# rvp-group/srrg2_slam_interfaces

Measured on AMD Instinct MI355X. Metric: icp_iterations_per_sec, higher is better.
Workload: dtype f32; 1 GPU; C2: SE(3) point-to-plane AlignerSlice, 100000-pt synthetic cloud pair per GPU, 10 ICP iterations per compute(), gated NN 0.25 m + normal gate, Cauchy 0.05; points=100000, alignments_total=1, all_success=True, last_status=0, last_num_inliers=99432, parallelism=single GPU

## Files before the change

srrg2_slam_interfaces_amd/csrc/aligner_host.hip:

```cpp
#include <algorithm>
#include <cmath>
#include <cstdio>
#include <cstdlib>
#include <chrono>
#include <cstring>
#include <string>
#include <vector>

#include "det_math.h"
#include "kernels.h"

#include "host_util.h"

namespace srrg2amd {
thread_local std::string g_err;
int fail(int code, const std::string& msg) {
  g_err = msg;
  return code;
}
}

namespace {

using srrg2amd::DevBuf;
// ... 802 lines not shown
      const Slice* sfc = a->slices[fc];
      const int sl     = tn.search_lists;
      const bool lists = sl >= 2 || (sl == 1 && K > 4) || (sl < 0 && (K > 4 || sfc->grid_computes >= 1 || sfc->lists_tried));
      small            = !lists && max_nm <= 384;
    }
  }
  const int fast_from = tn.fast_from_iteration;
  bool fuse = false;
  auto fast_ppt_of = [&](int k_launch) {
    return tn.fast_points_per_thread > 0 ? tn.fast_points_per_thread : (k_launch >= (fuse ? 16 : 64) ? 2 : 1);
  };
  const int fast_min = tn.fast_min_points;
  const bool fast_gather = tn.fast_gather >= 0 ? tn.fast_gather != 0 : K > 4;
  const bool fast_batch_queue = tn.fast_batch_queue != 0;
  const int lds_tile = pairs ? 0 : (tn.lds_tile >= 0 ? tn.lds_tile : (K > 4 ? 1 : 0));
  const int search_lists = tn.search_lists;
  const int search_team_knob = tn.search_team;
  std::vector<char> cnl((size_t) std::max(nslices, 1), 0);
  std::vector<SliceDev> sdev((size_t) nslices);
  int first_cue = -1;
  for (int si = 0; si < nslices; ++si) {
    Slice* s     = a->slices[si];
    SliceCtl& sc = C.slices[si];
    sc.kind                     = s->cfg.kind;
    sc.min_num_correspondences  = s->cfg.min_num_correspondences;
    sc.robust_kind              = s->cfg.robustifier;
    sc.robust_thr               = s->cfg.robustifier_chi_threshold;
    sc.gate                     = s->cfg.finder_max_distance;
    sc.has_prior                = s->has_prior ? 1 : 0;
    sc.prior_sets_initial_guess = s->cfg.prior_sets_initial_guess;
    std::memcpy(sc.prior_Z, s->prior_Z, sizeof(sc.prior_Z));
    std::memcpy(sc.prior_info, s->cfg.prior_information_diag, sizeof(sc.prior_info));
    sc.partials  = nullptr;
    sc.finder    = s->cfg.finder;
    sc.K0        = s->cfg.camera_matrix[0];
    sc.K4        = s->cfg.camera_matrix[4];
    sc.umax      = proj_extent(s->cfg.image_cols, s->cfg.camera_matrix[2]);
    sc.vmax      = proj_extent(s->cfg.image_rows, s->cfg.camera_matrix[5]);
    sc.depth_min = s->cfg.depth_min;
    sc.pinf_bits = nullptr;
    sc.ninf_bits = nullptr;
    if (s->cfg.kind == SRRG2_SLICE_PRIOR) continue;
    if (first_cue < 0) first_cue = si;
    int nm_max_s = 0;
    for (int k = 0; k < K; ++k) nm_max_s = std::max(nm_max_s, all[(size_t) si * K + k].nm);
    const int queue_min = tn.queue_min_points;
    const bool want_lists = search_lists >= 2 || (search_lists == 1 && K > 4) ||
                            (search_lists < 0 && (K > 4 || s->grid_computes >= 1 || s->lists_tried));
    if (!pairs) s->grid_computes++;
    if (s->cfg.finder == SRRG2_FINDER_NN_GATED && !small && want_lists && !pairs) {
      if ((rc = ensure_lists(a, s, 96LL << 20))) return rc;
      cnl[(size_t) si] = s->grid.list_R > 0 ? 1 : 0;
    }
    const bool use_queue = s->cfg.finder == SRRG2_FINDER_NN_GATED && nm_max_s >= queue_min && K <= 4 && !small && !cnl[(size_t) si] && !pairs;
    const bool fast_queue = s->cfg.finder == SRRG2_FINDER_NN_GATED && K > 4 && !small && fast_batch_queue && !pairs;
    s->fast_queue_only = fast_queue && !use_queue;
    const int nblocks    = PARTIAL_SLOTS;
    {
      const size_t cap_before = s->partials.cap;
      if ((rc = s->partials.reserve((size_t) 3 * K * nblocks * ACC_N))) return rc;
      if (s->partials.cap != cap_before) s->slots_zeroed = 0;
    }
    if (use_queue || fast_queue) {
      if ((rc = s->queue.reserve((size_t) std::max(s->nm_total, 1) * 10))) return rc;
      if ((rc = s->qcount.reserve((size_t) 2 * K))) return rc;
    }
    sc.qcount = (use_queue || fast_queue) ? s->qcount.p : nullptr;
    sc.qprobe_host = nullptr;
    sc.probs       = nullptr;
    if (use_queue) {
      if ((rc = ensure_pinned(s->qprobe_host, s->qprobe_cap, (size_t) 2 * K))) return rc;
      std::memset(s->qprobe_host, 0x7f, sizeof(int) * (size_t) 2 * K);
      sc.qprobe_host = s->qprobe_host;
      sc.probs       = a->probs.p + (size_t) si * K;
    }
    sc.partials  = s->partials.p;
    sc.pinf_bits = s->pinf.p;
    sc.ninf_bits = pairs ? a->pair_rows.p + PAIR_ROW_NINF : s->scalars.p + 7;
    sc.finf_bits = s->scalars.p + 10;
    sc.gcorr_off = nullptr;
    sc.nm_global = (a->reduce_fn && s->cfg.kind != SRRG2_SLICE_PRIOR) ? (int) a->shard_total : 0;
    SliceDev& d       = sdev[si];
    d.grid            = pairs ? GridDev{} : s->grid;
    d.mpts            = s->moving.p;
    d.mnrm            = s->moving_has_normals ? s->moving_nrm.p : nullptr;
    d.corr_fixed      = s->corr_fixed.p;
    d.corr_resp       = s->corr_resp.p;
    d.corr_stat       = s->corr_stat.p;
    d.prev_n          = s->prev_n.p;
    d.prev_pos        = s->prev_pos.p;
    d.prev_f          = s->prev_f.p;
    d.prev_m          = s->prev_m.p;
    d.dbg             = nullptr;
    if (!a->timeline_path.empty()) {
      const size_t nw = (size_t) K * ((nm_max_s + 255) / 256) * 4;
      if ((rc = s->dbg.reserve(32 * nw * 16))) return rc;
      HIP_TRY(hipMemsetAsync(s->dbg.p, 0, 32 * nw * 16 * sizeof(unsigned long long), a->stream));
      d.dbg = s->dbg.p;
    }
    d.partials        = s->partials.p;
    d.queue           = (use_queue || fast_queue) ? (void*) s->queue.p : nullptr;
    d.qcount          = (use_queue || fast_queue) ? s->qcount.p : nullptr;
    d.slice_idx       = si;
    d.robust_kind     = s->cfg.robustifier;
    d.robust_thr      = s->cfg.robustifier_chi_threshold;
    d.normal_cos      = s->cfg.finder_normal_cos;
    d.use_normal_gate = (s->cfg.finder_normal_cos > -1.f && (pairs ? a->pair_normals : s->fixed_has_normals) && s->moving_has_normals) ? 1 : 0;
    d.gather_prev     = (s->cfg.finder == SRRG2_FINDER_NN_GATED && fast_gather) ? 1 : 0;
    d.variable_kind   = a->kind;
    d.finder          = s->cfg.finder;
    d.factor          = s->cfg.kind;
    std::memcpy(d.K, s->cfg.camera_matrix, sizeof(d.K));
    d.rows            = s->cfg.image_rows;
    d.cols            = s->cfg.image_cols;
    d.depth_min       = s->cfg.depth_min;
    d.depth_max       = s->cfg.depth_max;
    d.gate            = s->cfg.finder_max_distance;
    d.fixed_org       = s->fixed_raw.p;
    d.fixed_org_nrm   = s->fixed_has_normals ? s->fixed_nrm_raw.p : nullptr;
    d.zbuf            = nullptr;
    d.zbuf_parity     = 0;
    d.gcorr = nullptr; d.gcorr_off = nullptr; d.gcorr_stat = nullptr;
    d.moving_raw      = s->moving_raw.p;
    if (s->cfg.finder == SRRG2_FINDER_CORRESPONDENCES) {
      if ((int) s->h_gcorr_off.size() != K + 1)
        return fail(SRRG2_E_STATE, "compute: given-correspondences slice without correspondences for every alignment");
      if (s->cfg.kind == SRRG2_SLICE_P2PLANE && !s->fixed_has_normals)
        return fail(SRRG2_E_STATE, "compute: point-to-plane slice without fixed normals");
      const int total = s->h_gcorr_off[(size_t) K];
      for (int k = 0; k < K; ++k) {
        const int nmk = all[(size_t) si * K + k].nm;
        for (int c = s->h_gcorr_off[(size_t) k]; c < s->h_gcorr_off[(size_t) k + 1]; ++c)
          if (s->h_gcorr[(size_t) c].fixed_idx < 0 || s->h_gcorr[(size_t) c].fixed_idx >= s->nf ||
              s->h_gcorr[(size_t) c].moving_idx < 0 || s->h_gcorr[(size_t) c].moving_idx >= nmk)
            return fail(SRRG2_E_INVALID, "compute: correspondence index out of range");
      }
      if ((rc = s->gcorr.reserve((size_t) std::max(total, 1)))) return rc;
      if ((rc = s->gcorr_off.reserve((size_t) K + 1))) return rc;
      if ((rc = s->gcorr_stat.reserve((size_t) std::max(total, 1)))) return rc;
      if (total > 0)
        HIP_TRY(hipMemcpyAsync(s->gcorr.p, s->h_gcorr.data(), sizeof(srrg2_correspondence) * (size_t) total,
                               hipMemcpyHostToDevice, a->stream));
      HIP_TRY(hipMemcpyAsync(s->gcorr_off.p, s->h_gcorr_off.data(), sizeof(int) * ((size_t) K + 1), hipMemcpyHostToDevice,
                             a->stream));
      HIP_TRY(hipStreamSynchronize(a->stream));
      d.gcorr      = s->gcorr.p;
      d.gcorr_off  = s->gcorr_off.p;
      d.gcorr_stat = s->gcorr_stat.p;
      sc.gcorr_off = s->gcorr_off.p;
    }
    if (s->cfg.finder == SRRG2_FINDER_PROJECTIVE) {
      if ((rc = s->zbuf.reserve((size_t) 2 * K * d.rows * d.cols))) return rc;
      d.zbuf = s->zbuf.p;
      HIP_TRY(hipMemsetAsync(s->zbuf.p, 0xff, (size_t) 2 * K * d.rows * d.cols * sizeof(unsigned long long), a->stream));
    }
    if (a->dim == 3)
      dm::se3_inverse(s->cfg.sensor_in_robot, d.Sinv);
    else
      dm::se2_inverse(s->cfg.sensor_in_robot, d.Sinv);
    std::memcpy(sc.Sinv, d.Sinv, sizeof(sc.Sinv));
  }
  if (K > 1 && first_cue >= 0 && !slice_offsets) {
    for (int si = 0; si < nslices; ++si)
      if (a->slices[si]->cfg.kind != SRRG2_SLICE_PRIOR && si != first_cue)
        return fail(SRRG2_E_UNSUPPORTED, "compute_batch supports one cue slice (plus prior slices)");
  }
// ... 1544 lines not shown
```

srrg2_slam_interfaces_amd/csrc/device_types.h:

```cpp
#pragma once
#include <hip/hip_runtime.h>
#include <stdint.h>

#include "../../include/srrg2_slam_amd.h"

#define ACC_N 32
#define PARTIAL_SLOTS 32
#define ACC_B 21
#define ACC_CHI_IN 27
#define ACC_CHI_OUT 28
#define ACC_N_IN 29
#define ACC_N_OUT 30
#define ACC_N_CORR 31
#define TERM_WINDOW_MAX 64
#define NO_MATCH 0x7fffffff

__host__ __device__ __forceinline__ constexpr int hidx(int a, int b) {
  return a * 6 - (a * (a - 1)) / 2 + (b - a);
}

struct GridDev {
  float ox, oy, oz;
  float h, inv_h;
  int nx, ny, nz;
  int rmax;
  int rfar_gate;
  float gate2;
  float gate2_ext;
  int n;
  const int* cell_start;
  const float4* pts;
  const float4* nrm;
  const int* pos_of;
  int list_R;
  const struct GridLists* lists;
};
struct GridLists {
  int R;
  int lnx, lny, lnz;
  const int* start;
  const uint4* ent;
  float cls_b2[14];
};
#define CNL_MAX_R 3
#ifndef CNL_ENTRY_MAX
#define CNL_ENTRY_MAX 16
#endif
#define CNL_MAX_CLASS 12

#define PUB_SLICE_GRANULES 64
#define PUB_G_KEXP 24
#define PUB_G_FLAGS 25
#define PUB_G_NSTATS 26
#define PUB_G_WCOUNT 27
#define PUB_G_NPASSES 28
#define PUB_G_X 32
#define PUB_FLAG_STOP 1u
#define PUB_FLAG_PHASE1 2u
#define PUB_FLAG_PRIOR 4u
#define PUB_EPOCH_REPLICAS 8
#define PUB_EPOCH_STRIDE 32
struct CtlParams;
struct FusedCtl {
  unsigned long long* pub;
  unsigned* pub_epoch;
  const CtlParams* ctl;
  srrg2_iteration_stats* stats;
  long long* prev_partials;
  long long* zero_partials;
  int epoch;
  int min_num_correspondences;
  int max_stats;
  int has_term;
  int first_round;
  int prior;
  int prior_mask;
  int nslices;
};

struct SliceDev {
  GridDev grid;
  const float4* mpts;
  const float4* mnrm;
  int* corr_fixed;
  float* corr_resp;
  uint8_t* corr_stat;
  float4* prev_f;
  float4* prev_n;
  int* prev_pos;
  float* prev_m;
  long long* partials;
  void* queue;
  int* qcount;
  int slice_idx;
  int robust_kind;
  float robust_thr;
  float normal_cos;
  int use_normal_gate;
  int gather_prev;
  int variable_kind;
  int finder;
  int factor;
  float K[9];
  int rows, cols;
  float depth_min, depth_max;
  float gate;
  const float4* fixed_org;
  const float4* fixed_org_nrm;
  unsigned long long* zbuf;
  int zbuf_parity;
  const srrg2_correspondence* gcorr;
  const int* gcorr_off;
  uint8_t* gcorr_stat;
  const float4* moving_raw;
  unsigned long long* dbg;
  int prob0;
  float Sinv[12];
// ... 99 lines not shown
```

srrg2_slam_interfaces_amd/csrc/kernels.hip:

```cpp
#include <cstdlib>
#include <algorithm>

#include "kernels.h"

#include <type_traits>

#include "det_math.h"

#include "device_util.h"

namespace {

#define FX_MAGIC 6755399441055744.0
#define FX_MAGIC_BITS 0x4338000000000000ll
__device__ __forceinline__ long long fx_bits(double biased) { return __double_as_longlong(biased) - FX_MAGIC_BITS; }

__device__ __forceinline__ unsigned long long key_min(unsigned long long a, unsigned long long b) {
  double r;
  asm("v_min_f64 %0, %1, %2" : "=v"(r) : "v"(__longlong_as_double((long long) a)), "v"(__longlong_as_double((long long) b)));
  return (unsigned long long) __double_as_longlong(r);
}

template <int DIM>
__device__ __forceinline__ float cand_d2(const float4 f, float qx, float qy, float qz) {
// ... 471 lines not shown

namespace {

#ifndef SRRG2_CNL_REDEAL
#define SRRG2_CNL_REDEAL 0
#endif
#ifdef SRRG2_CNL_STATS
__device__ unsigned long long g_cnl_stats[4 * 16];
#define CNL_STAT(k, v)                                                                                   \
  do {                                                                                                   \
    const unsigned long long v_ = (unsigned long long) (v);    \
    if ((threadIdx.x & 63) == 0) atomicAdd(&g_cnl_stats[(stat_it < 3 ? stat_it : 3) * 16 + (k)], v_);    \
  } while (0)
#else
#define CNL_STAT(k, v) do { } while (0)
#endif
constexpr int CNL_POOL = 512;

struct CnlWave {
  uint2 pool[CNL_POOL];
  unsigned long long key[64];
  unsigned b2[64];
  float q[3][64];
};

template <int DIM>
__device__ __forceinline__ void test_group_glb(const float4* __restrict__ pts, int j, int cnt, float qx, float qy, float qz,
                                               unsigned long long& bkey, float& b2) {
  if (cnt > 0) {
    const float4 a0 = pts[j], a1 = pts[j + 1], a2 = pts[j + 2], a3 = pts[j + 3];
    const float d0 = cand_d2<DIM>(a0, qx, qy, qz);
    float d1 = cand_d2<DIM>(a1, qx, qy, qz), d2 = cand_d2<DIM>(a2, qx, qy, qz), d3 = cand_d2<DIM>(a3, qx, qy, qz);
    unsigned i1 = (unsigned) __float_as_int(a1.w), i2 = (unsigned) __float_as_int(a2.w), i3 = (unsigned) __float_as_int(a3.w);
    d1 = cnt > 1 ? d1 : INFINITY;
    d2 = cnt > 2 ? d2 : INFINITY;
    d3 = cnt > 3 ? d3 : INFINITY;
    i1 = cnt > 1 ? i1 : (unsigned) NO_MATCH;
    i2 = cnt > 2 ? i2 : (unsigned) NO_MATCH;
    i3 = cnt > 3 ? i3 : (unsigned) NO_MATCH;
    b2   = __builtin_amdgcn_fmed3f(__uint_as_float((unsigned) (bkey >> 32)), b2, d0);
    bkey = key_min(bkey, ((unsigned long long) __float_as_uint(d0) << 32) | (unsigned) __float_as_int(a0.w));
    b2   = __builtin_amdgcn_fmed3f(__uint_as_float((unsigned) (bkey >> 32)), b2, d1);
    bkey = key_min(bkey, ((unsigned long long) __float_as_uint(d1) << 32) | i1);
    b2   = __builtin_amdgcn_fmed3f(__uint_as_float((unsigned) (bkey >> 32)), b2, d2);
    bkey = key_min(bkey, ((unsigned long long) __float_as_uint(d2) << 32) | i2);
    b2   = __builtin_amdgcn_fmed3f(__uint_as_float((unsigned) (bkey >> 32)), b2, d3);
    bkey = key_min(bkey, ((unsigned long long) __float_as_uint(d3) << 32) | i3);
  }
}

template <int DIM>
__device__ __forceinline__ void cnl_drain_pool(const float4* __restrict__ pts, CnlWave& w, int lane, int n, int stat_it = 3) {
  wave_lds_sync();
  CNL_STAT(6, n);
  for (int s0 = 0; s0 < n; s0 += 64) {
    CNL_STAT(7, 1);
    const int s     = s0 + lane;
    const bool have = s < n;
    uint2 it        = make_uint2(0u, 0u);
    if (have) it = w.pool[s];
    const int owner = (int) (it.y & 63u);
    int cnt         = have ? (int) (it.y >> 8) : 0;
    int j           = (int) it.x;
    const float qx = w.q[0][owner], qy = w.q[1][owner], qz = DIM == 3 ? w.q[2][owner] : 0.f;
    unsigned long long key = NO_KEY;
    float lb2              = INFINITY;
    while (__any(cnt > 0)) {
      CNL_STAT(8, 1);
      CNL_STAT(9, __popcll(__ballot(cnt > 0)));
      test_group_glb<DIM>(pts, j, cnt, qx, qy, qz, key, lb2);
      j += 4;
      cnt -= 4;
    }
    if (have) {
      const unsigned long long old   = atomicMin(&w.key[owner], key);
      const unsigned long long loser = old > key ? old : key;
      const unsigned l2              = min((unsigned) (loser >> 32), __float_as_uint(lb2));
      atomicMin(&w.b2[owner], l2);
    }
  }
  wave_lds_sync();
}

template <int DIM, int TEAM>
__device__ __forceinline__ void cnl_phase0(const GridDev& g, const GridLists& gl, int lane, bool need, float qx, float qy, float qz,
                                           float r2box, float gfar, unsigned long long& bkey, float& b2, float& L, int& e,
                                           int& eend, int stat_it = 3) {
  const int R  = gl.R;
  const int tl = lane & (TEAM - 1);
  const int cx = cell_coord(qx, g.ox, g.inv_h);
  const int cy = cell_coord(qy, g.oy, g.inv_h);
  const int cz = DIM == 3 ? cell_coord(qz, g.oz, g.inv_h) : 0;
  const int lx = cx + R, ly = cy + R, lz = DIM == 3 ? cz + R : 0;
  const bool inl = need && lx >= 0 && lx < gl.lnx && ly >= 0 && ly < gl.lny && lz >= 0 && lz < gl.lnz;
  e = 0;
  eend = 0;
  if (inl) {
    const int lc = (lz * gl.lny + ly) * gl.lnx + lx;
    e            = gl.start[lc];
    eend         = gl.start[lc + 1];
  }
  bkey = NO_KEY;
  b2   = INFINITY;
  L    = fminf(r2box, gfar);
  {
    const bool p0 = e < eend;
    uint4 h0      = make_uint4(0u, 0u, 0u, 0u);
    if (p0) h0 = gl.ent[e];
    int j = (int) h0.x + 4 * tl, cnt = p0 ? (int) (h0.y & 15u) + 1 - 4 * tl : 0;
    CNL_STAT(10, __popcll(__ballot(need)));
    while (__any(cnt > 0)) {
      CNL_STAT(1, 1);
      CNL_STAT(2, __popcll(__ballot(cnt > 0)));
      test_group_glb<DIM>(g.pts, j, cnt, qx, qy, qz, bkey, b2);
      j += 4 * TEAM;
      cnt -= 4 * TEAM;
    }
#pragma unroll
    for (int off = 1; off < TEAM; off <<= 1) {
      const unsigned long long ok = __shfl_xor(bkey, off);
      const float ob2             = __shfl_xor(b2, off);
      const unsigned long long lo = ok < bkey ? ok : bkey, hi = ok < bkey ? bkey : ok;
      b2   = fminf(fminf(b2, ob2), __uint_as_float((unsigned) (hi >> 32)));
      bkey = lo;
    }
    if (p0) {
      ++e;
      if (key_idx(bkey) != NO_MATCH) {
        const float rb = (sqrtf(key_best(bkey)) + (PAD_CAP + PAD_MIN) * g.h) * 1.00001f;
        L              = fminf(L, rb * rb);
      }
    }
  }
}

template <int DIM, int TEAM>
__device__ __forceinline__ void cnl_phaseAB(const GridDev& g, const GridLists& gl, CnlWave& w, int lane, float qx, float qy,
                                            float qz, unsigned long long& bkey, float& b2, float L, int e, int eend,
                                            int stat_it = 3) {
  const int R  = gl.R;
  const int tl = lane & (TEAM - 1);
  const int owner_lane = lane - tl;
  const float ux0 = (qx - g.ox) * g.inv_h, uy0 = (qy - g.oy) * g.inv_h, uz0 = DIM == 3 ? (qz - g.oz) * g.inv_h : 0.f;
  const int cx = cell_coord(qx, g.ox, g.inv_h);
  const int cy = cell_coord(qy, g.oy, g.inv_h);
  const int cz = DIM == 3 ? cell_coord(qz, g.oz, g.inv_h) : 0;
  if (tl == 0) {
    w.key[lane]  = bkey;
    w.b2[lane]   = __float_as_uint(b2);
    w.q[0][lane] = qx;
    w.q[1][lane] = qy;
    if (DIM == 3) w.q[2][lane] = qz;
  }
  const float Lc  = L * 1.00002f;
  const float Lcc = ((Lc * g.inv_h) * g.inv_h * 1.0001f) * 256.f;
  int mmax = -1;
#pragma unroll
  for (int m = 0; m <= CNL_MAX_CLASS; ++m) mmax += gl.cls_b2[m] <= Lc ? 1 : 0;
  const float fR = (float) R;
  const float mx = 0.011f + fabsf(ux0) * 1e-6f, my = 0.011f + fabsf(uy0) * 1e-6f, mz = 0.011f + fabsf(uz0) * 1e-6f;
  const float ux = ux0 - (float) cx, uy = uy0 - (float) cy, uz = uz0 - (float) cz;
  const float cax = ((fR + ux) + mx) * 16.f, cbx = ((fR + ux) - mx) * 16.f;
  const float cay = ((fR + uy) + my) * 16.f, cby = ((fR + uy) - my) * 16.f;
  const float caz = ((fR + uz) + mz) * 16.f, cbz = ((fR + uz) - mz) * 16.f;
  int pool_n = 0;
  e += 4 * tl;
  CNL_STAT(0, 1);
  CNL_STAT(11, __popcll(__ballot(e < eend)));
  while (__any(e < eend)) {
    CNL_STAT(3, 1);
    CNL_STAT(4, __popcll(__ballot(e < eend)));
    uint4 hd[4];
#pragma unroll
    for (int k = 0; k < 4; ++k) {
      hd[k] = make_uint4(0u, 0xf0u, 0u, 0u);
      if (e + k < eend) hd[k] = gl.ent[e + k];
    }
    bool stop = e >= eend;
#pragma unroll
    for (int k = 0; k < 4; ++k) {
      const unsigned code = hd[k].y;
      stop = stop || (int) ((code >> 4) & 15u) > mmax;
      const unsigned blo = hd[k].z, bhi = hd[k].w;
      const float lx_ = (float) (blo & 255u), ly_ = (float) ((blo >> 8) & 255u);
      const float hx_ = (float) (bhi & 255u), hy_ = (float) ((bhi >> 8) & 255u);
      const float tx = fmaxf(fmaxf(lx_ - cax, cbx - hx_), 0.f);
      const float ty = fmaxf(fmaxf(ly_ - cay, cby - hy_), 0.f);
      float d2c      = __fmaf_rn(ty, ty, tx * tx);
      if (DIM == 3) {
        const float lz_ = (float) ((blo >> 16) & 255u), hz_ = (float) ((bhi >> 16) & 255u);
        const float tz  = fmaxf(fmaxf(lz_ - caz, cbz - hz_), 0.f);
        d2c             = __fmaf_rn(tz, tz, d2c);
      }
      const bool surv             = !stop && !(d2c > Lcc);
      const unsigned long long bm = __ballot(surv);
      if (surv) {
        const int slot = pool_n + (int) __builtin_amdgcn_mbcnt_hi((unsigned) (bm >> 32), __builtin_amdgcn_mbcnt_lo((unsigned) bm, 0u));
        w.pool[slot]   = make_uint2(hd[k].x, (unsigned) owner_lane | (((code & 15u) + 1u) << 8));
      }
      pool_n += __popcll(bm);
    }
    e = stop ? eend : min(e + 4 * TEAM, eend);
    if (pool_n > CNL_POOL - 256) {
      cnl_drain_pool<DIM>(g.pts, w, lane, pool_n, stat_it);
      pool_n = 0;
    }
  }
  cnl_drain_pool<DIM>(g.pts, w, lane, pool_n, stat_it);
  bkey = w.key[owner_lane];
  b2   = __uint_as_float(w.b2[owner_lane]);
}

template <int DIM, int TEAM>
__device__ __forceinline__ void cnl_search(const GridDev& g, const GridLists& gl, CnlWave& w, int lane, bool need, float qx,
                                           float qy, float qz, float r2box, float gfar, unsigned long long& bkey, float& b2,
                                           float& L, int stat_it = 3) {
  int e, eend;
  cnl_phase0<DIM, TEAM>(g, gl, lane, need, qx, qy, qz, r2box, gfar, bkey, b2, L, e, eend, stat_it);
  cnl_phaseAB<DIM, TEAM>(g, gl, w, lane, qx, qy, qz, bkey, b2, L, e, eend, stat_it);
}

}

template <int DIM, bool PLANE>
__device__ __forceinline__ void finish_point(const SliceDev& S, const float* T, int rk, float thr, float kk, double scale,
                                             bool inrange, bool active, int gi, int oi, const float4 p, float qx, float qy,
                                             float qz, float best, int bidx, int bpos, float excl, bool kept,
                                             const float4 kept_f, const float4 kept_n, const float4 early_nm, bool have_nm,
                                             long long (&acc)[ACC_N]) {
  constexpr int D    = DIM == 3 ? 6 : 3;
  constexpr int ROWS = PLANE ? 1 : DIM;
  const GridDev& g   = S.grid;
  int match     = -1;
  float resp    = 0.f;
  uint8_t fstat = SRRG2_FACTOR_SUPPRESSED;
  float4 fm     = make_float4(0.f, 0.f, 0.f, __int_as_float(NO_MATCH));
  float4 nf     = make_float4(0.f, 0.f, 0.f, 0.f);
  if (inrange) {
    if (active) {
      bool found = bidx != NO_MATCH && best <= g.gate2;
      if (!kept && bidx != NO_MATCH) bpos = g.pos_of[bidx];
      if (bidx != NO_MATCH && (PLANE || S.use_normal_gate))
        nf = kept ? kept_n : g.nrm[bpos];
      if (bidx != NO_MATCH) fm = kept ? kept_f : g.pts[bpos];
      if (found && S.use_normal_gate) {
        const float4 nm = have_nm ? early_nm : S.mnrm[gi];
        float dot;
        if constexpr (DIM == 3) {
          float rx = (T[0] * nm.x + T[1] * nm.y) + T[2] * nm.z;
          float ry = (T[4] * nm.x + T[5] * nm.y) + T[6] * nm.z;
          float rz = (T[8] * nm.x + T[9] * nm.y) + T[10] * nm.z;
          dot      = (nf.x * rx + nf.y * ry) + nf.z * rz;
        } else {
          float rx = T[0] * nm.x + T[1] * nm.y;
          float ry = T[4] * nm.x + T[5] * nm.y;
          dot      = nf.x * rx + nf.y * ry;
        }
        if (!(dot > S.normal_cos)) found = false;
      }
      if (found) {
        match          = bidx;
        resp           = best;
        const float4 f = fm;
        float J[ROWS][D];
        float e[ROWS];
        if constexpr (DIM == 3) {
          float m[ROWS][3];
          if (PLANE) {
            e[0]    = (nf.x * (qx - f.x) + nf.y * (qy - f.y)) + nf.z * (qz - f.z);
            m[0][0] = (T[0] * nf.x + T[4] * nf.y) + T[8] * nf.z;
            m[0][1] = (T[1] * nf.x + T[5] * nf.y) + T[9] * nf.z;
            m[0][2] = (T[2] * nf.x + T[6] * nf.y) + T[10] * nf.z;
          } else {
            const float q[3]  = {qx, qy, qz};
            const float ff[3] = {f.x, f.y, f.z};
#pragma unroll
            for (int r = 0; r < ROWS; ++r) {
              e[r]    = q[r] - ff[r];
              m[r][0] = T[r * 4 + 0];
              m[r][1] = T[r * 4 + 1];
              m[r][2] = T[r * 4 + 2];
            }
          }
#pragma unroll
          for (int r = 0; r < ROWS; ++r) {
            J[r][0]     = m[r][0];
            J[r][1]     = m[r][1];
            J[r][2]     = m[r][2];
            J[r][D - 3] = kk * (p.y * m[r][2] - p.z * m[r][1]);
            J[r][D - 2] = kk * (p.z * m[r][0] - p.x * m[r][2]);
            J[r][D - 1] = kk * (p.x * m[r][1] - p.y * m[r][0]);
          }
        } else {
          float m[ROWS][2];
          if (PLANE) {
            e[0]    = nf.x * (qx - f.x) + nf.y * (qy - f.y);
            m[0][0] = T[0] * nf.x + T[4] * nf.y;
            m[0][1] = T[1] * nf.x + T[5] * nf.y;
          } else {
            const float q[2]  = {qx, qy};
            const float ff[2] = {f.x, f.y};
#pragma unroll
// ... 2093 lines not shown
  }
  const float thr    = S.robust_thr;
  const float kk     = S.variable_kind == SRRG2_SE3_QUAT_RIGHT ? 2.f : 1.f;
  const GridDev& g   = S.grid;
  const float gfar   = g.gate2_ext;
  const int rfar     = g.rmax;
  const float gate_r = S.gate * 1.000001f;
  const bool ngate   = S.use_normal_gate != 0;
  const bool use_q   = !FUSED && S.queue != nullptr && st->qmode[S.slice_idx] != 0;
  const int lane     = threadIdx.x & 63;
  const int wid      = threadIdx.x >> 6;
  union FastWaveLds {
    CnlWave cnl;
    int coop[288];
  };
  __shared__ FastWaveLds fast_lds[4];
  int* const coop_lds_w = fast_lds[wid].coop;

  auto linearize = [&](auto first, long long (&acc)[ACC_N], bool valid, const float4 pk, const float4 fk, const float4 nk,
                       const float4 nmk, float qx, float qy, float qz, float best) {
    bool found = valid && __float_as_int(fk.w) != NO_MATCH && best <= g.gate2;
    if (ngate) {
      float dot;
      if constexpr (DIM == 3) {
        const float rx = (T[0] * nmk.x + T[1] * nmk.y) + T[2] * nmk.z;
        const float ry = (T[4] * nmk.x + T[5] * nmk.y) + T[6] * nmk.z;
        const float rz = (T[8] * nmk.x + T[9] * nmk.y) + T[10] * nmk.z;
        dot            = (nk.x * rx + nk.y * ry) + nk.z * rz;
      } else {
        const float rx = T[0] * nmk.x + T[1] * nmk.y;
        const float ry = T[4] * nmk.x + T[5] * nmk.y;
        dot            = nk.x * rx + nk.y * ry;
      }
      found = found && dot > S.normal_cos;
    }
    float J[ROWS][D], e[ROWS];
    point_rows<DIM, PLANE>(T, kk, pk, qx, qy, qz, fk, nk, J, e);
    (void) factor_accumulate_flat<D, ROWS, decltype(first)::value>(J, e, found, rk, thr, scale, acc);
  };

  long long acc[ACC_N];

  float4 p[PPT], pf[PPT], pnm[PPT], pn[PPT];
  float pm[PPT];
  int gi_[PPT];
  bool inr[PPT];
#pragma unroll
  for (int k = 0; k < PPT; ++k) {
    const int i = (tile * PPT + k) * 256 + (int) threadIdx.x;
    inr[k]      = i < pd.nm;
    gi_[k]      = pd.moff + (inr[k] ? i : 0);
    int ppos    = -1;
    p[k]        = S.mpts[gi_[k]];
    pm[k]       = S.prev_m[gi_[k]];
    pf[k]       = make_float4(0.f, 0.f, 0.f, __int_as_float(NO_MATCH));
    pn[k]       = make_float4(0.f, 0.f, 0.f, 0.f);
    pnm[k]      = make_float4(0.f, 0.f, 0.f, 0.f);
    if (GATHER) {
      ppos = S.prev_pos[gi_[k]];
    } else {
      pf[k] = S.prev_f[gi_[k]];
      if (PLANE || ngate) pn[k] = S.prev_n[gi_[k]];
    }
    if (ngate) pnm[k] = S.mnrm[gi_[k]];
    if (GATHER && ppos >= 0 && ppos < g.n) {
      pf[k] = g.pts[ppos];
      if (PLANE || ngate) pn[k] = g.nrm[ppos];
    }
  }
  if constexpr (FUSED) {
    pass_view_fused<DIM, FUSED == 2>(S, states, prob, pv);
    if (pv.stop || tile * (256 * PPT) >= pd.nm) return;
    load_T(pv.T, T);
    load_T(pv.Tprev, Tprev);
    scale = dm::pow2(pv.kexp);
    rk    = (pv.phase1 && S.robust_kind != SRRG2_ROBUST_NONE) ? (int) SRRG2_ROBUST_CLAMP : S.robust_kind;
  }

  float open_ball2[PPT];
  bool any_open = false;
  auto search_open = [&](float (&sbest)[PPT], int (&sidx)[PPT], float (&sexcl)[PPT], int (&spos)[PPT]) {
  #pragma unroll
    for (int k = 0; k < PPT; ++k) {
      sbest[k] = INFINITY; sexcl[k] = 0.f; sidx[k] = NO_MATCH; spos[k] = 0;
      const bool open = open_ball2[k] >= 0.f;
      if (!__ballot(open)) continue;
      float qx = 0.f, qy = 0.f, qz = 0.f;
      if (open) transform_point<DIM>(T, p[k], qx, qy, qz);
      if (g.list_R > 0 && __popcll(__ballot(open)) > 4) {
        unsigned long long skey;
        float sb2, sL;
        cnl_search<DIM, 1>(g, *g.lists, fast_lds[wid].cnl, lane, open, qx, qy, qz, open_ball2[k], gfar, skey, sb2, sL);
        if (open) {
          sbest[k] = key_best(skey);
          sidx[k]  = key_idx(skey);
          sexcl[k] = sqrtf(fminf(sb2, fminf(sL, g.gate2_ext))) * 0.99999f;
        }
        continue;
      }
      bool open_k = open;
      if constexpr (PPT == 1) {
        if (!(g.list_R > 0) && __popcll(__ballot(open)) > 4) {
          unsigned long long lkey = NO_KEY;
          float lb2 = INFINITY, lc2 = INFINITY;
          if (open)
            scan_radius1<DIM>(g, qx, qy, qz, cell_coord(qx, g.ox, g.inv_h), cell_coord(qy, g.oy, g.inv_h),
                              DIM == 3 ? cell_coord(qz, g.oz, g.inv_h) : 0, open_ball2[k], lkey, lb2, lc2);
          const float b2_1 = bound2_of(1, g.h);
          if (open && key_idx(lkey) != NO_MATCH && key_best(lkey) <= gfar && key_best(lkey) <= b2_1) {
            sbest[k] = key_best(lkey);
            sidx[k]  = key_idx(lkey);
            sexcl[k] = sqrtf(fminf(fminf(lb2, lc2), b2_1)) * 0.99999f;
            open_k   = false;
          }
        }
      }
      const int r2 = open_ball2[k] <= bound2_of(2, g.h) ? 2 : max(rfar, 3);
      unsigned long long near = __ballot(open_k && r2 == 2);
      while (near) {
        int src[4];
  #pragma unroll
        for (int t = 0; t < 4; ++t) {
          src[t] = near ? __ffsll((long long) near) - 1 : -1;
          near &= near - 1;
        }
        const int team = lane >> 4;
        const int mine = team == 0 ? src[0] : (team == 1 ? src[1] : (team == 2 ? src[2] : src[3]));
        const int from = mine >= 0 ? mine : lane;
        const float sqx = __shfl(qx, from), sqy = __shfl(qy, from), sqz = __shfl(qz, from), sball = __shfl(open_ball2[k], from);
        const int scx = cell_coord(sqx, g.ox, g.inv_h), scy = cell_coord(sqy, g.oy, g.inv_h);
        const int scz = DIM == 3 ? cell_coord(sqz, g.oz, g.inv_h) : 0;
        float wbest, wexcl2;
        int widx, wpos;
        coop_scan<DIM, 16>(g, lane, coop_lds_w, sqx, sqy, sqz, scx, scy, scz, mine >= 0 ? 2 : -1, sball, wbest, widx, wpos, wexcl2);
  #pragma unroll
        for (int t = 0; t < 4; ++t) {
          const float rb = __shfl(wbest, 16 * t), re = __shfl(wexcl2, 16 * t);
          const int ri = __shfl(widx, 16 * t), rp = __shfl(wpos, 16 * t);
          if (lane == src[t]) {
            sbest[k] = rb;
            sidx[k]  = ri;
            spos[k]  = rp;
            sexcl[k] = sqrtf(re) * 0.99999f;
          }
        }
      }
      unsigned long long todo = __ballot(open_k && r2 != 2);
      while (todo) {
        const int src = __ffsll((long long) todo) - 1;
        todo &= todo - 1;
        const float sqx = __shfl(qx, src), sqy = __shfl(qy, src), sqz = __shfl(qz, src);
        const int scx = cell_coord(sqx, g.ox, g.inv_h), scy = cell_coord(sqy, g.oy, g.inv_h);
        const int scz = DIM == 3 ? cell_coord(sqz, g.oz, g.inv_h) : 0;
        float wbest, wexcl2;
        int widx, wpos;
        coop_scan<DIM, 64>(g, lane, coop_lds_w, sqx, sqy, sqz, scx, scy, scz, __shfl(r2, src), __shfl(open_ball2[k], src),
                           wbest, widx, wpos, wexcl2);
        if (lane == src) {
          sbest[k] = wbest;
          sidx[k]  = widx;
          spos[k]  = wpos;
          sexcl[k] = sqrtf(wexcl2) * 0.99999f;
        }
      }
    }
  };
  constexpr bool defer = PPT == 1 && FUSED;
  float d_qx = 0.f, d_qy = 0.f, d_qz = 0.f, d_best = INFINITY;
  bool d_valid = false;
#pragma unroll
  for (int k = 0; k < PPT; ++k) {
    const bool active = inr[k] && finite3(p[k].x, p[k].y, p[k].z);
    float qx, qy, qz, px, py, pz;
    transform_point<DIM>(T, p[k], qx, qy, qz);
    transform_point<DIM>(Tprev, p[k], px, py, pz);
    const float ex = qx - px, ey = qy - py, ez = qz - pz;
    const float dl   = __builtin_amdgcn_sqrtf((ex * ex + ey * ey) + ez * ez);
    const bool hasp  = __float_as_int(pf[k].w) != NO_MATCH;
    unsigned long long k1 = NO_KEY;
    test_candidate<DIM>(pf[k], qx, qy, qz, true, k1);
    const float best = key_best(k1);
    const float d1   = __builtin_amdgcn_sqrtf(best);
    const float rhs  = pm[k] * 0.99999f;
    const bool ca   = hasp && (d1 * 1.00001f + dl * 1.00001f < rhs);
    const bool cc   = !hasp && pm[k] > 0.f && (gate_r * 1.00001f + dl * 1.00001f < rhs);
    const bool have = active && (ca || cc);
    const float excl = pm[k] * 0.9999999f - dl * 1.00001f;
    const float pad  = fminf(2.f * dl, PAD_CAP * g.h) + PAD_MIN * g.h;
    const float rr   = (d1 + pad) * 1.00001f;
    const float r2box = hasp ? fminf(rr * rr, gfar) : gfar;
    open_ball2[k]     = (active && !have) ? r2box : -1.f;
    any_open |= active && !have;
#ifdef SRRG2_PASS_TIMELINE
    if constexpr (FUSED) {
      if (active && !have && S.fc.epoch >= 0 && S.fc.epoch < 16 && blockIdx.x == 0) {
        unsigned long long* c = &g_pass_ts[((size_t) S.fc.epoch * 512 + 500) * 8];
        const float gap = (pm[k] - d1) / g.h;
        atomicAdd(&c[0], 1ull);
        if (!hasp) atomicAdd(&c[1], 1ull);
        else if (gap < 1e-4f) atomicAdd(&c[2], 1ull);
        else if (gap < 0.0202f) atomicAdd(&c[3], 1ull);
        else atomicAdd(&c[4], 1ull);
        if (dl > 1e-3f * g.h) atomicAdd(&c[5], 1ull);
        if (pm[k] <= 0.f) atomicAdd(&c[6], 1ull);
      }
    }
#endif
    if constexpr (defer) {
      d_qx = qx; d_qy = qy; d_qz = qz; d_best = best; d_valid = have && ca;
    } else if (k == 0) {
      linearize(std::true_type{}, acc, have && ca, p[k], pf[k], pn[k], pnm[k], qx, qy, qz, best);
    } else {
      linearize(std::false_type{}, acc, have && ca, p[k], pf[k], pn[k], pnm[k], qx, qy, qz, best);
    }
    if (have) S.prev_m[gi_[k]] = excl;
  }
  if constexpr (defer) {
    {
      if (__any(any_open)) {
        float sbest[PPT], sexcl[PPT];
        int sidx[PPT], spos[PPT];
        search_open(sbest, sidx, sexcl, spos);
        const bool open = open_ball2[0] >= 0.f;
        const bool same = open && sidx[0] != NO_MATCH && sidx[0] == __float_as_int(pf[0].w);
        if (open && !same) {
          pf[0] = make_float4(0.f, 0.f, 0.f, __int_as_float(NO_MATCH));
          pn[0] = make_float4(0.f, 0.f, 0.f, 0.f);
          if (sidx[0] != NO_MATCH) {
            spos[0] = g.pos_of[sidx[0]];
            pf[0]   = g.pts[spos[0]];
            if (PLANE || ngate) pn[0] = g.nrm[spos[0]];
          }
          S.prev_pos[gi_[0]] = sidx[0] != NO_MATCH ? spos[0] : -1;
          if (!GATHER) {
            S.prev_f[gi_[0]] = pf[0];
            if (PLANE || ngate) S.prev_n[gi_[0]] = pn[0];
          }
        }
        if (open) {
          S.prev_m[gi_[0]] = sexcl[0];
          d_best  = sbest[0];
          d_valid = true;
        }
      }
      linearize(std::true_type{}, acc, d_valid, p[0], pf[0], pn[0], pnm[0], d_qx, d_qy, d_qz, d_best);
      block_reduce_store_biased<4>(acc, S.partials, prob, tile, PPT);
      if constexpr (FUSED) PASS_TS(S.fc.epoch, 3);
      return;
    }
  }
  if (use_q) {
#pragma unroll
    for (int k = 0; k < PPT; ++k) {
      const bool open               = open_ball2[k] >= 0.f;
      const unsigned long long need = __ballot(open);
      if (!need) continue;
      const int r2 = open_ball2[k] <= bound2_of(2, g.h) ? 2 : max(rfar, 3);
      const unsigned long long need_near = __ballot(open && r2 == 2);
      const unsigned long long need_far  = need & ~need_near;
      int base_near = 0, base_far = 0;
      if (lane == 0) {
        if (need_near) base_near = atomicAdd(&S.qcount[2 * prob], __popcll(need_near));
        if (need_far) base_far = atomicAdd(&S.qcount[2 * prob + 1], __popcll(need_far));
      }
      base_near = __shfl(base_near, 0);
      base_far  = __shfl(base_far, 0);
      if (open) {
        const unsigned long long below = (1ull << lane) - 1ull;
        QEntry q;
        q.i = (tile * PPT + k) * 256 + (int) threadIdx.x;
        q.r2 = r2; q.best = INFINITY; q.bidx = NO_MATCH; q.bpos = 0;
        transform_point<DIM>(T, p[k], q.qx, q.qy, q.qz);
        q.ball2 = open_ball2[k]; q.pad_ = 0;
        QEntry* qbase = reinterpret_cast<QEntry*>(S.queue) + pd.moff;
        if (r2 == 2)
          qbase[base_near + __popcll(need_near & below)] = q;
        else
          qbase[pd.nm - 1 - (base_far + __popcll(need_far & below))] = q;
      }
    }
  }
  block_reduce_store_biased<4, 1>(acc, S.partials, prob, tile, PPT);
  if (use_q || !__any(any_open)) {
    block_reduce_store_biased<4, 2>(acc, S.partials, prob, tile, PPT);
    if constexpr (FUSED) PASS_TS(S.fc.epoch, 3);
    return;
  }

  float sbest[PPT], sexcl[PPT];
  int sidx[PPT], spos[PPT];
  search_open(sbest, sidx, sexcl, spos);
  long long acc2[ACC_N];
#pragma unroll
  for (int k = 0; k < PPT; ++k) {
    const bool open = open_ball2[k] >= 0.f;
    float4 fk = make_float4(0.f, 0.f, 0.f, __int_as_float(NO_MATCH)), nk = make_float4(0.f, 0.f, 0.f, 0.f);
    bool same = false;
    if constexpr (PPT == 1) same = open && sidx[k] != NO_MATCH && sidx[k] == __float_as_int(pf[k].w);
    if (same) {
      fk = pf[k];
      nk = pn[k];
    } else if (open && sidx[k] != NO_MATCH) {
      spos[k] = g.pos_of[sidx[k]];
      fk      = g.pts[spos[k]];
      if (PLANE || ngate) nk = g.nrm[spos[k]];
    }
    float qx, qy, qz;
    transform_point<DIM>(T, p[k], qx, qy, qz);
    if (k == 0)
      linearize(std::true_type{}, acc2, open, p[k], fk, nk, pnm[k], qx, qy, qz, sbest[k]);
    else
      linearize(std::false_type{}, acc2, open, p[k], fk, nk, pnm[k], qx, qy, qz, sbest[k]);
    if (open) {
      S.prev_m[gi_[k]] = sexcl[k];
      if (!same) {
        S.prev_pos[gi_[k]] = sidx[k] != NO_MATCH ? spos[k] : -1;
        if (!GATHER) {
          S.prev_f[gi_[k]] = fk;
          if (PLANE || ngate) S.prev_n[gi_[k]] = nk;
        }
      }
    }
  }
  block_reduce_store_biased<1>(acc2, S.partials, prob, tile, PPT);
  if constexpr (FUSED) PASS_TS_ANY(S.fc.epoch, 4);
  block_reduce_store_biased<4, 2>(acc, S.partials, prob, tile, PPT);
  if constexpr (FUSED) PASS_TS(S.fc.epoch, 3);
}

template <int DIM, bool PLANE, int PPT, bool GATHER, int FUSED>
__global__ __launch_bounds__(256) void k_icp_step_fast(SliceDev S, const ProblemDev* __restrict__ probs,
                                                       ProblemState* __restrict__ states) {
  icp_step_fast_body<DIM, PLANE, PPT, GATHER, FUSED>(S, probs, states);
}
template <int DIM, bool PLANE, int PPT, bool GATHER>
__global__ __launch_bounds__(256) void k_icp_step_fast_pairs(SliceDev S, const GridDev* __restrict__ grids,
                                                             const ProblemDev* __restrict__ probs, ProblemState* __restrict__ states) {
  S.grid = grids[blockIdx.y + S.prob0];
  icp_step_fast_body<DIM, PLANE, PPT, GATHER, 0>(S, probs, states);
}
template <int DIM, bool PLANE, int TEAM, int FUSED>
__device__ __forceinline__ void cnl_pass_body(const SliceDev& S, const GridLists& GL, const ProblemDev* __restrict__ probs,
                                              ProblemState* __restrict__ states, const CtlParams* Ci = nullptr,
                                              const InitInline* inl = nullptr, const InitBatch* bat = nullptr) {
  constexpr int NW  = 4;
  constexpr int PPB = NW * 64 / TEAM;
  const int prob    = (FUSED ? blockIdx.x : blockIdx.y) + S.prob0;
  PassView pv;
  if constexpr (!FUSED) {
    pass_view_legacy(S, &states[prob], pv);
    if (pv.stop) return;
  } else if constexpr (FUSED != 3) {
    PASS_TS(S.fc.epoch, 0);
    fused_control_if_due<DIM, FUSED == 2>(S, states, prob);
  }
  ProblemDev pd;
  if constexpr (FUSED == 3) {
    if (bat)
      pd = bat->pd[prob - Ci->prob0];
    else
      pd = inl->pd[S.slice_idx];
  } else {
    pd = probs[prob];
  }
  const int tile      = FUSED ? blockIdx.y : blockIdx.x;
  const bool tail_wg = FUSED == 3 && tile == (int) gridDim.y - 1;
  if (tile * PPB >= pd.nm && (!FUSED || (FUSED == 3 ? !tail_wg : tile != 0))) return;
  float T[12], Tprev[12];
  double scale;
  int rk;
  bool use_prior;
  if constexpr (!FUSED) {
    load_T(pv.T, T);
    load_T(pv.Tprev, Tprev);
    scale     = dm::pow2(pv.kexp);
    rk        = (pv.phase1 && S.robust_kind != SRRG2_ROBUST_NONE) ? (int) SRRG2_ROBUST_CLAMP : S.robust_kind;
    use_prior = pv.prior;
  } else {
    use_prior = S.fc.prior != 0;
  }
  const float thr    = S.robust_thr;
  const float kk     = S.variable_kind == SRRG2_SE3_QUAT_RIGHT ? 2.f : 1.f;
  const GridDev& g   = S.grid;
  const float gfar = use_prior ? g.gate2_ext : g.gate2;

  __shared__ CnlWave wlds[NW];

// ... 2041 lines not shown
```

Baseline: 59780 iterations/s.

## Add ball-bounded cell-list search for sparse reopened queries in fused ICP

Adds a new cnl_search_ball path for waves with at most four reopened queries. It uses precomputed cell lists with box pruning against the query's ball radius, instead of the general phase0/phaseAB search, and returns the grid position of the best match directly. The prune setup and box-distance code move into shared helpers. Callers now skip the pos_of indirection when a position is already known. The aim is to cut search and gather cost in the common late-ICP case where few points need re-search, at the cost of extra code, register pressure and a new host flag (search_lists != 3) that controls it.

```diff
diff --git a/srrg2_slam_interfaces_amd/csrc/aligner_host.hip b/srrg2_slam_interfaces_amd/csrc/aligner_host.hip
--- a/srrg2_slam_interfaces_amd/csrc/aligner_host.hip
+++ b/srrg2_slam_interfaces_amd/csrc/aligner_host.hip
@@ -908,6 +908,7 @@
     sc.nm_global = (a->reduce_fn && s->cfg.kind != SRRG2_SLICE_PRIOR) ? (int) a->shard_total : 0;
     SliceDev& d       = sdev[si];
     d.grid            = pairs ? GridDev{} : s->grid;
+    d.grid.list_ball  = tn.search_lists != 3 ? 1 : 0;
     d.mpts            = s->moving.p;
     d.mnrm            = s->moving_has_normals ? s->moving_nrm.p : nullptr;
     d.corr_fixed      = s->corr_fixed.p;
diff --git a/srrg2_slam_interfaces_amd/csrc/device_types.h b/srrg2_slam_interfaces_amd/csrc/device_types.h
--- a/srrg2_slam_interfaces_amd/csrc/device_types.h
+++ b/srrg2_slam_interfaces_amd/csrc/device_types.h
@@ -33,6 +33,7 @@
   const float4* nrm;
   const int* pos_of;
   int list_R;
+  int list_ball;
   const struct GridLists* lists;
 };
 struct GridLists {
diff --git a/srrg2_slam_interfaces_amd/csrc/kernels.hip b/srrg2_slam_interfaces_amd/csrc/kernels.hip
--- a/srrg2_slam_interfaces_amd/csrc/kernels.hip
+++ b/srrg2_slam_interfaces_amd/csrc/kernels.hip
@@ -577,6 +577,46 @@
   wave_lds_sync();
 }
 
+struct CnlPrune {
+  float Lcc;
+  int mmax;
+  float cax, cbx, cay, cby, caz, cbz;
+};
+template <int DIM>
+__device__ __forceinline__ CnlPrune cnl_prune_of(const GridDev& g, const GridLists& gl, float qx, float qy, float qz, float L) {
+  CnlPrune P;
+  const float ux0 = (qx - g.ox) * g.inv_h, uy0 = (qy - g.oy) * g.inv_h, uz0 = DIM == 3 ? (qz - g.oz) * g.inv_h : 0.f;
+  const int cx = cell_coord(qx, g.ox, g.inv_h);
+  const int cy = cell_coord(qy, g.oy, g.inv_h);
+  const int cz = DIM == 3 ? cell_coord(qz, g.oz, g.inv_h) : 0;
+  const float Lc = L * 1.00002f;
+  P.Lcc  = ((Lc * g.inv_h) * g.inv_h * 1.0001f) * 256.f;
+  P.mmax = -1;
+#pragma unroll
+  for (int m = 0; m <= CNL_MAX_CLASS; ++m) P.mmax += gl.cls_b2[m] <= Lc ? 1 : 0;
+  const float fR = (float) gl.R;
+  const float mx = 0.011f + fabsf(ux0) * 1e-6f, my = 0.011f + fabsf(uy0) * 1e-6f, mz = 0.011f + fabsf(uz0) * 1e-6f;
+  const float ux = ux0 - (float) cx, uy = uy0 - (float) cy, uz = uz0 - (float) cz;
+  P.cax = ((fR + ux) + mx) * 16.f; P.cbx = ((fR + ux) - mx) * 16.f;
+  P.cay = ((fR + uy) + my) * 16.f; P.cby = ((fR + uy) - my) * 16.f;
+  P.caz = ((fR + uz) + mz) * 16.f; P.cbz = ((fR + uz) - mz) * 16.f;
+  return P;
+}
+template <int DIM>
+__device__ __forceinline__ float cnl_box_d2(const CnlPrune& P, unsigned blo, unsigned bhi) {
+  const float lx_ = (float) (blo & 255u), ly_ = (float) ((blo >> 8) & 255u);
+  const float hx_ = (float) (bhi & 255u), hy_ = (float) ((bhi >> 8) & 255u);
+  const float tx = fmaxf(fmaxf(lx_ - P.cax, P.cbx - hx_), 0.f);
+  const float ty = fmaxf(fmaxf(ly_ - P.cay, P.cby - hy_), 0.f);
+  float d2c      = __fmaf_rn(ty, ty, tx * tx);
+  if (DIM == 3) {
+    const float lz_ = (float) ((blo >> 16) & 255u), hz_ = (float) ((bhi >> 16) & 255u);
+    const float tz  = fmaxf(fmaxf(lz_ - P.caz, P.cbz - hz_), 0.f);
+    d2c             = __fmaf_rn(tz, tz, d2c);
+  }
+  return d2c;
+}
+
 template <int DIM, int TEAM>
 __device__ __forceinline__ void cnl_phase0(const GridDev& g, const GridLists& gl, int lane, bool need, float qx, float qy, float qz,
                                            float r2box, float gfar, unsigned long long& bkey, float& b2, float& L, int& e,
@@ -633,13 +673,8 @@
 __device__ __forceinline__ void cnl_phaseAB(const GridDev& g, const GridLists& gl, CnlWave& w, int lane, float qx, float qy,
                                             float qz, unsigned long long& bkey, float& b2, float L, int e, int eend,
                                             int stat_it = 3) {
-  const int R  = gl.R;
   const int tl = lane & (TEAM - 1);
   const int owner_lane = lane - tl;
-  const float ux0 = (qx - g.ox) * g.inv_h, uy0 = (qy - g.oy) * g.inv_h, uz0 = DIM == 3 ? (qz - g.oz) * g.inv_h : 0.f;
-  const int cx = cell_coord(qx, g.ox, g.inv_h);
-  const int cy = cell_coord(qy, g.oy, g.inv_h);
-  const int cz = DIM == 3 ? cell_coord(qz, g.oz, g.inv_h) : 0;
   if (tl == 0) {
     w.key[lane]  = bkey;
     w.b2[lane]   = __float_as_uint(b2);
@@ -647,17 +682,9 @@
     w.q[1][lane] = qy;
     if (DIM == 3) w.q[2][lane] = qz;
   }
-  const float Lc  = L * 1.00002f;
-  const float Lcc = ((Lc * g.inv_h) * g.inv_h * 1.0001f) * 256.f;
-  int mmax = -1;
-#pragma unroll
-  for (int m = 0; m <= CNL_MAX_CLASS; ++m) mmax += gl.cls_b2[m] <= Lc ? 1 : 0;
-  const float fR = (float) R;
-  const float mx = 0.011f + fabsf(ux0) * 1e-6f, my = 0.011f + fabsf(uy0) * 1e-6f, mz = 0.011f + fabsf(uz0) * 1e-6f;
-  const float ux = ux0 - (float) cx, uy = uy0 - (float) cy, uz = uz0 - (float) cz;
-  const float cax = ((fR + ux) + mx) * 16.f, cbx = ((fR + ux) - mx) * 16.f;
-  const float cay = ((fR + uy) + my) * 16.f, cby = ((fR + uy) - my) * 16.f;
-  const float caz = ((fR + uz) + mz) * 16.f, cbz = ((fR + uz) - mz) * 16.f;
+  const CnlPrune P = cnl_prune_of<DIM>(g, gl, qx, qy, qz, L);
+  const int mmax   = P.mmax;
+  const float Lcc  = P.Lcc;
   int pool_n = 0;
   e += 4 * tl;
   CNL_STAT(0, 1);
@@ -676,17 +703,7 @@
     for (int k = 0; k < 4; ++k) {
       const unsigned code = hd[k].y;
       stop = stop || (int) ((code >> 4) & 15u) > mmax;
-      const unsigned blo = hd[k].z, bhi = hd[k].w;
-      const float lx_ = (float) (blo & 255u), ly_ = (float) ((blo >> 8) & 255u);
-      const float hx_ = (float) (bhi & 255u), hy_ = (float) ((bhi >> 8) & 255u);
-      const float tx = fmaxf(fmaxf(lx_ - cax, cbx - hx_), 0.f);
-      const float ty = fmaxf(fmaxf(ly_ - cay, cby - hy_), 0.f);
-      float d2c      = __fmaf_rn(ty, ty, tx * tx);
-      if (DIM == 3) {
-        const float lz_ = (float) ((blo >> 16) & 255u), hz_ = (float) ((bhi >> 16) & 255u);
-        const float tz  = fmaxf(fmaxf(lz_ - caz, cbz - hz_), 0.f);
-        d2c             = __fmaf_rn(tz, tz, d2c);
-      }
+      const float d2c             = cnl_box_d2<DIM>(P, hd[k].z, hd[k].w);
       const bool surv             = !stop && !(d2c > Lcc);
       const unsigned long long bm = __ballot(surv);
       if (surv) {
@@ -713,6 +730,91 @@
   int e, eend;
   cnl_phase0<DIM, TEAM>(g, gl, lane, need, qx, qy, qz, r2box, gfar, bkey, b2, L, e, eend, stat_it);
   cnl_phaseAB<DIM, TEAM>(g, gl, w, lane, qx, qy, qz, bkey, b2, L, e, eend, stat_it);
+}
+
+template <int DIM>
+__device__ __forceinline__ void cnl_search_ball(const GridDev& g, const GridLists& gl, CnlWave& w, int lane, bool have, float sqx,
+                                                float sqy, float sqz, float sball, float gfar, float& wbest, int& widx, int& wpos,
+                                                float& wexcl2) {
+  const int tl      = lane & 15;
+  const int tshift  = lane & 48;
+  uint2* const pool = w.pool + 2 * tshift;
+  const int R  = gl.R;
+  const int lx = cell_coord(sqx, g.ox, g.inv_h) + R, ly = cell_coord(sqy, g.oy, g.inv_h) + R;
+  const int lz = DIM == 3 ? cell_coord(sqz, g.oz, g.inv_h) + R : 0;
+  const bool inl = have && lx >= 0 && lx < gl.lnx && ly >= 0 && ly < gl.lny && lz >= 0 && lz < gl.lnz;
+  int e = 0, eend = 0;
+  if (inl) {
+    const int lc = (lz * gl.lny + ly) * gl.lnx + lx;
+    e            = gl.start[lc];
+    eend         = gl.start[lc + 1];
+  }
+  const float L    = fminf(sball, gfar);
+  const CnlPrune P = cnl_prune_of<DIM>(g, gl, sqx, sqy, sqz, L);
+  unsigned long long key = NO_KEY;
+  float lb2              = INFINITY;
+  int lpos               = 0;
+  while (__any(e < eend)) {
+    uint4 hd[2];
+#pragma unroll
+    for (int k = 0; k < 2; ++k) {
+      hd[k] = make_uint4(0u, 0xf0u, 0u, 0u);
+      if (e + 16 * k + tl < eend) hd[k] = gl.ent[e + 16 * k + tl];
+    }
+    int n       = 0;
+    bool beyond = false;
+#pragma unroll
+    for (int k = 0; k < 2; ++k) {
+      const unsigned code = hd[k].y;
+      const bool far_     = (int) ((code >> 4) & 15u) > P.mmax;
+      beyond              = beyond || far_;
+      const bool surv     = !far_ && !(cnl_box_d2<DIM>(P, hd[k].z, hd[k].w) > P.Lcc);
+      const unsigned bm   = (unsigned) (__ballot(surv) >> tshift) & 0xffffu;
+      if (surv) pool[n + __popc(bm & ((1u << tl) - 1u))] = make_uint2(hd[k].x, (code & 15u) + 1u);
+      n += __popc(bm);
+    }
+    e = ((__ballot(beyond) >> tshift) & 0xffffull) ? eend : min(e + 32, eend);
+    wave_lds_sync();
+    for (int s0 = 0; __any(s0 < 4 * n); s0 += 16) {
+      const int s = s0 + tl;
+      int j = 0, cnt = 0;
+      if (s < 4 * n) {
+        const uint2 it = pool[s >> 2];
+        j              = (int) it.x + 4 * (s & 3);
+        cnt            = (int) it.y - 4 * (s & 3);
+      }
+      if (cnt > 0) {
+        float4 a[4];
+#pragma unroll
+        for (int c = 0; c < 4; ++c) a[c] = g.pts[j + c];
+#pragma unroll
+        for (int c = 0; c < 4; ++c) {
+          const float d      = cnt > c ? cand_d2<DIM>(a[c], sqx, sqy, sqz) : INFINITY;
+          const unsigned idx = cnt > c ? (unsigned) __float_as_int(a[c].w) : (unsigned) NO_MATCH;
+          lb2 = __builtin_amdgcn_fmed3f(key_best(key), lb2, d);
+          const unsigned long long nk = key_min(key, ((unsigned long long) __float_as_uint(d) << 32) | idx);
+          lpos = nk != key ? j + c : lpos;
+          key  = nk;
+        }
+      }
+    }
+    wave_lds_sync();
+  }
+  unsigned long long kmin = key;
+  float v                 = lb2;
+#pragma unroll
+  for (int off = 1; off < 16; off <<= 1) {
+    const unsigned long long ok = __shfl_xor(kmin, off);
+    const float ov              = __shfl_xor(v, off);
+    const unsigned long long lo = ok < kmin ? ok : kmin, hi = ok < kmin ? kmin : ok;
+    v    = fminf(fminf(v, ov), key_best(hi));
+    kmin = lo;
+  }
+  const unsigned wm = (unsigned) (__ballot(key == kmin) >> tshift) & 0xffffu;
+  wpos   = __shfl(lpos, tshift + (wm ? __ffs((int) wm) - 1 : 0));
+  wbest  = key_best(kmin);
+  widx   = key_idx(kmin);
+  wexcl2 = fminf(v, fminf(L, g.gate2_ext));
 }
 
 }
@@ -2972,11 +3074,39 @@
   auto search_open = [&](float (&sbest)[PPT], int (&sidx)[PPT], float (&sexcl)[PPT], int (&spos)[PPT]) {
   #pragma unroll
     for (int k = 0; k < PPT; ++k) {
-      sbest[k] = INFINITY; sexcl[k] = 0.f; sidx[k] = NO_MATCH; spos[k] = 0;
+      sbest[k] = INFINITY; sexcl[k] = 0.f; sidx[k] = NO_MATCH; spos[k] = -1;
       const bool open = open_ball2[k] >= 0.f;
       if (!__ballot(open)) continue;
       float qx = 0.f, qy = 0.f, qz = 0.f;
       if (open) transform_point<DIM>(T, p[k], qx, qy, qz);
+      if (PPT == 1 && FUSED != 0 && g.list_R > 0 && g.list_ball && __popcll(__ballot(open)) <= 4) {
+        unsigned long long few = __ballot(open);
+        int src[4];
+  #pragma unroll
+        for (int t = 0; t < 4; ++t) {
+          src[t] = few ? __ffsll((long long) few) - 1 : -1;
+          few &= few - 1;
+        }
+        const int team = lane >> 4;
+        const int mine = team == 0 ? src[0] : (team == 1 ? src[1] : (team == 2 ? src[2] : src[3]));
+        const int from = mine >= 0 ? mine : lane;
+        const float sqx = __shfl(qx, from), sqy = __shfl(qy, from), sqz = __shfl(qz, from), sball = __shfl(open_ball2[k], from);
+        float wbest, wexcl2;
+        int widx, wpos;
+        cnl_search_ball<DIM>(g, *g.lists, fast_lds[wid].cnl, lane, mine >= 0, sqx, sqy, sqz, sball, gfar, wbest, widx, wpos, wexcl2);
+  #pragma unroll
+        for (int t = 0; t < 4; ++t) {
+          const float rb = __shfl(wbest, 16 * t), re = __shfl(wexcl2, 16 * t);
+          const int ri = __shfl(widx, 16 * t), rp = __shfl(wpos, 16 * t);
+          if (lane == src[t]) {
+            sbest[k] = rb;
+            sidx[k]  = ri;
+            spos[k]  = rp;
+            sexcl[k] = sqrtf(re) * 0.99999f;
+          }
+        }
+        continue;
+      }
       if (g.list_R > 0 && __popcll(__ballot(open)) > 4) {
         unsigned long long skey;
         float sb2, sL;
@@ -3026,11 +3156,10 @@
   #pragma unroll
         for (int t = 0; t < 4; ++t) {
           const float rb = __shfl(wbest, 16 * t), re = __shfl(wexcl2, 16 * t);
-          const int ri = __shfl(widx, 16 * t), rp = __shfl(wpos, 16 * t);
+          const int ri = __shfl(widx, 16 * t);
           if (lane == src[t]) {
             sbest[k] = rb;
             sidx[k]  = ri;
-            spos[k]  = rp;
             sexcl[k] = sqrtf(re) * 0.99999f;
           }
         }
@@ -3049,7 +3178,6 @@
         if (lane == src) {
           sbest[k] = wbest;
           sidx[k]  = widx;
-          spos[k]  = wpos;
           sexcl[k] = sqrtf(wexcl2) * 0.99999f;
         }
       }
@@ -3117,8 +3245,8 @@
           pf[0] = make_float4(0.f, 0.f, 0.f, __int_as_float(NO_MATCH));
           pn[0] = make_float4(0.f, 0.f, 0.f, 0.f);
           if (sidx[0] != NO_MATCH) {
-            spos[0] = g.pos_of[sidx[0]];
-            pf[0]   = g.pts[spos[0]];
+            if (spos[0] < 0) spos[0] = g.pos_of[sidx[0]];
+            pf[0] = g.pts[spos[0]];
             if (PLANE || ngate) pn[0] = g.nrm[spos[0]];
           }
           S.prev_pos[gi_[0]] = sidx[0] != NO_MATCH ? spos[0] : -1;
@@ -3191,8 +3319,8 @@
       fk = pf[k];
       nk = pn[k];
     } else if (open && sidx[k] != NO_MATCH) {
-      spos[k] = g.pos_of[sidx[k]];
-      fk      = g.pts[spos[k]];
+      if (spos[k] < 0) spos[k] = g.pos_of[sidx[k]];
+      fk = g.pts[spos[k]];
       if (PLANE || ngate) nk = g.nrm[spos[k]];
     }
     float qx, qy, qz;
```

Result: no change. 60900 iterations/s, median of 3 (+1.9%).
